# tesseract-robotics/trajopt

Hardware: NVIDIA H100
Metric: converged trajectories/sec (7-DOF x 30 wp, batch 1024) (higher is better)
Workload: dtype f64

## Files before the change

### trajopt_b200/csrc/kernels.h

```cpp
#pragma once
#include "device_types.cuh"

namespace tb200 {
struct EvalExtra;
struct SolveCtl;
using SolveKernelFn = void (*)(DevProblem, EvalExtra, SolveCtl);
using EvalKernelFn = void (*)(DevProblem, EvalExtra, int, const double*);
SolveKernelFn solve_kernel_for(int D, bool pair_rows, bool sing);
EvalKernelFn eval_kernel_for(int D, bool sing);
int eval_debug_prof(unsigned long long* out, int reset);
constexpr int kQpProfSlots = 32;
int qp_debug_prof(unsigned long long* out, int reset);
}
```

### trajopt_b200/csrc/qp_cta_kernel.cuh

```cuda
#pragma once
#include "device_types.cuh"
#include "joint_terms.cuh"

namespace tb200 {

#ifdef TB200_PROFILE
static __device__ unsigned long long g_prof[32];
#define PROF_T0() const long long prof_t0_ = clock64()
#define PROF_ADD(slot) do { if (q.tid == 0) atomicAdd(&g_prof[slot], (unsigned long long)(clock64() - prof_t0_)); } while (0)
#define PROF_COUNT(slot) do { if (q.tid == 0) atomicAdd(&g_prof[slot], 1ull); } while (0)
#define PROF_ADD2(slot, slot2) do { if (q.tid == 0) { const unsigned long long d_ = clock64() - prof_t0_; \
    atomicAdd(&g_prof[slot], d_); atomicAdd(&g_prof[slot2], d_); } } while (0)
#else
#define PROF_T0()
#define PROF_ADD(slot)
#define PROF_COUNT(slot)
#define PROF_ADD2(slot, slot2)
#endif
#if defined(TB200_PROFILE) && defined(TB200_PROFILE_CHECK)
#define PROF_CHK_T0() long long pc_ = clock64()
#define PROF_CHK(slot) do { const long long n_ = clock64(); if (q.tid == 0) atomicAdd(&g_prof[slot], (unsigned long long)(n_ - pc_)); pc_ = n_; } while (0)
#else
#define PROF_CHK_T0()
#define PROF_CHK(slot)
#endif

constexpr int kQpThreads = 256;
constexpr int kQpThreadsC = 256;
constexpr double kOsqpInf = 1e30;
constexpr double kMinScaling = 1e-4, kMaxScaling = 1e4;
constexpr double kVerifyTol = 1e-9;
constexpr int kVerifyRounds = 3;
constexpr double kRhoMin = 1e-6, kRhoMax = 1e6, kRhoTol = 1e-4, kRhoEqOverIneq = 1e3;
enum { QPS_UNSOLVED = 0, QPS_SOLVED = 1, QPS_SOLVED_INACC = 2, QPS_PINF = 3, QPS_PINF_INACC = 4, QPS_DINF = 5,
       QPS_DINF_INACC = 6, QPS_MAXITER = 7, QPS_NONCVX = 8 };

__device__ __forceinline__ double limit_scaling(double v) {
  v = v < kMinScaling ? 1.0 : v;
  return v > kMaxScaling ? kMaxScaling : v;
}
// ... 1441 lines not shown
      }
      v_x = xn;
      v_z = zn;
      v_y += dy;
    }
    __syncthreads();
    PROF_ADD(3);
  }
  if (has_var) {
    q.x[vi] = v_x;
    q.zb[vi] = v_z;
    q.yb[vi] = v_y;
  }
  __syncthreads();
}

template <int NB, int PAIR>
__device__ __noinline__ void admm_block_pinv(const QpCtx& q, const double rho_aux_in, const int n_iter, const int keep_last) {
  constexpr int CNc = PAIR ? ((NB > 3) ? NB : 3) : ((NB / 2 > 3) ? NB / 2 : 3);
  constexpr int kPre = 8;
  constexpr int QN = 3 * NB;
  constexpr int kRowThreads = 64;
  extern __shared__ double sm[];
#ifdef TB200_PROFILE
  const long long prof_entry_ = clock64();
#endif
  const int tid = q.tid, N = q.N, Np = q.Np, nrows = q.nrows, RS = q.RS;
  const double sigma = q.sigma, alpha = q.alpha, oma = 1.0 - q.alpha, rho = q.rho, rho_eq = q.rho_eq, rho_aux = rho_aux_in;
  const double inv_rho_aux = 1.0 / rho_aux, inv_rho = 1.0 / rho, inv_rho_eq = 1.0 / rho_eq;
  double* const v1 = sm + (q.v1 - q.smbase);
  double* const w = sm + (q.w - q.smbase);
  double* const rows = sm + (q.rows - q.smbase);
  const int* const rints = reinterpret_cast<const int*>(sm + (reinterpret_cast<const double*>(q.rints) - q.smbase));
  const int* const colent = reinterpret_cast<const int*>(sm + (reinterpret_cast<const double*>(q.colent) - q.smbase));
  double* const dxs = q.scratch;
  double* const dyb = q.scratch + Np;
  const int M = q.M, PR = q.pl.PR, nS = q.pl.nS, ZS = q.pl.ZS, HO = q.pl.HO, WS = q.pl.WS;
  const double* const fbase = sm + (q.SA - q.smbase);
  const bool upper = tid >= kQpThreads - kRowThreads;
  const bool prow = tid < PR;
  const int pp = prow ? tid / QN : 0, plr = prow ? tid % QN : 0;
  const int pb0 = pp * 4 * NB, pvar = pb0 + plr;
  const int pn = ((M - 4 * pp) < 3 ? (M - 4 * pp) : 3) * NB;
  const int xl_off = (pp > 0) ? (4 * pp - 1) * NB : 0;
  const int xr_off = (4 * pp + 3 < M) ? (4 * pp + 3) * NB : 0;
  const unsigned a_wrow = smem_u32(fbase + q.pl.wo + (prow ? tid : 0) * WS);
  const unsigned a_b = smem_u32(v1 + pb0), a_xl = smem_u32(w + xl_off), a_xr = smem_u32(w + xr_off);
  const bool swork = tid >= PR && tid < PR + 2 * nS;
  const int sw = swork ? tid - PR : 0, srow = sw >> 1, half = sw & 1;
// ... 61 lines not shown
      const double xt = w[vi];
      const double xn = alpha * xt + oma * v_x;
      const double zr = alpha * (v_beta * xt) + oma * v_z;
      double zn = zr + v_y * v_irb;
      zn = fmin(fmax(zn, v_lb), v_ub);
      const double dy = v_rb * (zr - zn);
      if (keep_steps) {
        v_dx = xn - v_x;
        v_dy = dy;
        dxs[vi] = v_dx;
        dyb[vi] = v_dy;
      }
      v_x = xn;
      v_z = zn;
      v_y += dy;
    }
  };

  if (!upper) {
    double pi[QN];
#pragma unroll
    for (int j = 0; j < QN; ++j) pi[j] = prow ? q.pi_g[j * PR + tid] : 0.0;
    bar();
#ifdef TB200_PROFILE
    if (tid == 0) atomicAdd(&g_prof[21], (unsigned long long)(clock64() - prof_entry_));
#endif
    for (int it = 0; it < n_iter; ++it) {
      const bool keep_steps = keep_last && it == n_iter - 1;
      { PROF_T0(); build_rhs(); PROF_ADD(1); }
      {
        PROF_T0();
        PROF_CHK_T0();
        bar();
        PROF_CHK(4);
        double y = 0.0;
        if (prow) {
          double y0 = 0.0, y1 = 0.0;
#pragma unroll
          for (int j = 0; j < QN; j += 2) {
            double2 bb = make_double2(0.0, 0.0);
            if (j < pn) bb = lds_v2_at(a_b + j * 8);
            y0 += pi[j] * bb.x;
            y1 += pi[j + 1] * bb.y;
          }
          y = y0 + y1;
        }
        sep_half();
        PROF_CHK(14);
        bar();
        PROF_CHK(15);
        if (prow) {
          double t0 = 0.0, t1 = 0.0;
#pragma unroll
          for (int t = 0; t < NB; t += 2) {
            const double2 wl = lds_v2_at(a_wrow + t * 8), wr = lds_v2_at(a_wrow + (NB + t) * 8);
            const double2 xl = lds_v2_at(a_xl + t * 8), xr = lds_v2_at(a_xr + t * 8);
            t0 += wl.x * xl.x + wr.x * xr.x;
            t1 += wl.y * xl.y + wr.y * xr.y;
          }
          w[pvar] = y - (t0 + t1);
        }
        bar();
        PROF_CHK(9);
        PROF_ADD(2);
      }
      {
        PROF_T0();
        var_update(keep_steps);
        bar();
        PROF_ADD(3);
      }
    }
  } else {
    for (int r = kQpThreads - 1 - tid; r < nrows; r += kRowThreads)
      admm_row_entry<CNc>(rows + r * RS, rows + r * RS + 2 * CNc, sigma, rho_aux);
    bar();
    for (int it = 0; it < n_iter; ++it) {
      const bool keep_steps = keep_last && it == n_iter - 1;
      build_rhs();
      bar();
      sep_half();
      bar();
      bar();
      for (int r = kQpThreads - 1 - tid; r < nrows; r += kRowThreads)
        admm_row_update<CNc>(rows + r * RS, rows + r * RS + 2 * CNc, rints + r * RI_NINTS, w, sigma, alpha, oma, rho_aux,
                             inv_rho_aux);
      var_update(keep_steps);
      bar();
    }
  }
  if (has_var) {
    q.x[vi] = v_x;
    q.zb[vi] = v_z;
    q.yb[vi] = v_y;
// ... 37 lines not shown
    static_assert(CHK_PA0 == 14 && CHK_DA1 == 18, "vals[] follows ChkQ");
    __syncwarp();
#pragma unroll
    for (int k = 0; k < kChkHash; ++k) {
      double v = vals[k];
      if ((kChkSumMask >> k) & 1u) {
#pragma unroll
        for (int off = 16; off > 0; off >>= 1) v += __shfl_xor_sync(0xffffffffu, v, off);
      } else {
        v = warp_max_norm(v);
      }
      vals[k] = v;
    }
    for (int off = 16; off > 0; off >>= 1) h += __shfl_xor_sync(0xffffffffu, h, off);
    if ((tid & 31) == 0) {
      double* const chk = sm + (q.tmp - q.smbase);
      const int wid = tid >> 5;
#pragma unroll
      for (int k = 0; k < kChkHash; ++k) chk[k * 8 + wid] = vals[k];
      reinterpret_cast<unsigned long long*>(chk + kChkHash * 8)[wid] = h;
    }
    __syncthreads();
  }
}

enum SoaF { S_U0 = 0, S_U1, S_B0, S_B1, S_LO, S_UP, S_QA0, S_QA1, S_WRR, S_IWRR, S_G0, S_G1, S_IDEN, S_UPA0, S_UPA1,
            S_Z, S_Y, S_XA0, S_XA1, S_ZA0, S_ZA1, S_YA0, S_YA1, S_RA0, S_RA1, S_AS };
__host__ __device__ inline size_t qp_soa_doubles(int max_rows, int CN) {
  const size_t rsd = (static_cast<size_t>(max_rows) + 31) & ~static_cast<size_t>(31);
  return rsd * (S_AS + CN) + (rsd * (3 + CN) + 1) / 2 + static_cast<size_t>(max_rows) * CN + 8;
}
template <int NB, int PAIR>
__device__ __noinline__ void admm_block_soa(const QpCtx& q, const double rho_aux_in, const int n_iter, const int keep_last) {
  constexpr int CNc = PAIR ? ((NB > 3) ? NB : 3) : ((NB / 2 > 3) ? NB / 2 : 3);
  const int N = q.N, Np = q.Np, tid = q.tid, nrows = q.nrows;
  const double sigma = q.sigma, alpha = q.alpha, oma = 1.0 - q.alpha, rho = q.rho, rho_eq = q.rho_eq, rho_aux = rho_aux_in;
  const double inv_rho_aux = 1.0 / rho_aux, inv_rho = 1.0 / rho, inv_rho_eq = 1.0 / rho_eq;
  double* const dxs = q.scratch;
  double* const dyb = q.scratch + Np;
  const int RSd = (nrows + 31) & ~31;
  double* const sd = q.soa;
  int* const si = reinterpret_cast<int*>(sd + static_cast<size_t>(RSd) * (S_AS + CNc));
  double* const ct = sd + static_cast<size_t>(RSd) * (S_AS + CNc) + (static_cast<size_t>(RSd) * (3 + CNc) + 1) / 2 + 1;
  const int nnz = q.colptr[Np];
  PROF_T0();
  for (int i = tid; i < N; i += kQpThreads)
// ... 116 lines not shown
      const double xt = q.w[i];
      const double xn = alpha * xt + oma * q.x[i];
      const double zr = alpha * (beta * xt) + oma * q.zb[i];
      double zn = zr + q.yb[i] * irb;
      zn = fmin(fmax(zn, lb), ub);
      const double dy = rb * (zr - zn);
      if (keep_steps) {
        dxs[i] = xn - q.x[i];
        dyb[i] = dy;
      }
      q.x[i] = xn;
      q.zb[i] = zn;
      q.yb[i] += dy;
    }
    __syncthreads();
    PROF_SOA(3);
  }
}

__device__ inline void qp_scale(QpCtx& q, const QpSettings& st, int n_aux_total) {
  double *qs = q.qs, *lbs = q.lbs, *ubs = q.ubs;
  const int N = q.N, tid = q.tid, HB = 2 * q.D, W = HB + 1;
  double* Eb = q.zb;
  q.c = 1.0;
  for (int i = tid; i < q.Np; i += kQpThreads) {
    q.Dz[i] = 1.0;
    Eb[i] = 1.0;
  }
  for (int r = tid; r < q.nrows; r += kQpThreads) {
    double* F = q.F(r);
    F[R_E] = F[R_DA0] = F[R_DA1] = F[R_EA0] = F[R_EA1] = 1.0;
  }
  __syncthreads();
  for (int pass = 0; pass < st.scaling; ++pass) {
    for (int r = tid; r < q.nrows; r += kQpThreads) {
      double* R = q.R(r);
      double* F = q.F(r);
      const int* I = q.I(r);
      const int base = I[RI_BASE], cnt = I[RI_CNT], stride = I[RI_STRIDE], aux = I[RI_AUX];
      const double E = F[R_E];
      double rn = 0.0;
      for (int k = 0; k < cnt; ++k) rn = fmax(rn, fabs(E * R[k] * q.Dz[base + k * stride]));
      double dt0 = 1.0, dt1 = 1.0, et0 = 1.0, et1 = 1.0;
      if (aux >= 1) {
        const double ua = fabs(E * F[R_DA0]), ba = fabs(F[R_EA0] * F[R_DA0]);
        rn = fmax(rn, ua);
        dt0 = 1.0 / sqrt(limit_scaling(fmax(ua, ba)));
        et0 = 1.0 / sqrt(limit_scaling(ba));
      }
      if (aux == 2) {
        const double ua = fabs(E * F[R_DA1]), ba = fabs(F[R_EA1] * F[R_DA1]);
        rn = fmax(rn, ua);
        dt1 = 1.0 / sqrt(limit_scaling(fmax(ua, ba)));
        et1 = 1.0 / sqrt(limit_scaling(ba));
      }
      F[R_RA0] = 1.0 / sqrt(limit_scaling(rn));
      F[R_RA1] = E;
      F[R_DA0] *= dt0;
      F[R_DA1] *= dt1;
      F[R_EA0] *= et0;
      F[R_EA1] *= et1;
    }
    __syncthreads();
    for (int i = tid; i < N; i += kQpThreads) {
      double m = 0.0;
      for (int t = 0; t < q.n_band; ++t) {
        const int k = q.band_offs[t];
        if (k <= i) m = fmax(m, fabs(q.c * q.Dz[i] * q.Pband[i * W + k] * q.Dz[i - k]));
        if (k >= 1 && i + k < N) m = fmax(m, fabs(q.c * q.Dz[i] * q.Pband[(i + k) * W + k] * q.Dz[i + k]));
      }
      const double bn = fabs(Eb[i] * q.Dz[i]);
      m = fmax(m, bn);
      for (int e = q.colptr[i]; e < q.colptr[i + 1]; ++e) {
        const int ent = q.colent[e], r = ent >> 5, k = ent & 31;
        const double* R = q.R(r);
        m = fmax(m, fabs(R[2 * q.CN + R_RA1] * R[k] * q.Dz[i]));
      }
      q.v1[i] = 1.0 / sqrt(limit_scaling(m));
      Eb[i] *= 1.0 / sqrt(limit_scaling(bn));
    }
    __syncthreads();
    for (int i = tid; i < N; i += kQpThreads) q.Dz[i] *= q.v1[i];
    for (int r = tid; r < q.nrows; r += kQpThreads) {
      double* F = q.F(r);
      F[R_E] = F[R_RA1] * F[R_RA0];
    }
    __syncthreads();
    double csum = 0.0, qn = 0.0;
    for (int i = tid; i < N; i += kQpThreads) {
      double m = 0.0;
      for (int t = 0; t < q.n_band; ++t) {
        const int k = q.band_offs[t];
        if (k <= i) m = fmax(m, fabs(q.c * q.Dz[i] * q.Pband[i * W + k] * q.Dz[i - k]));
        if (k >= 1 && i + k < N) m = fmax(m, fabs(q.c * q.Dz[i] * q.Pband[(i + k) * W + k] * q.Dz[i + k]));
      }
      csum += m;
      qn = fmax(qn, fabs(q.c * q.Dz[i] * qs[i]));
    }
    for (int r = tid; r < q.nrows; r += kQpThreads) {
      const double* F = q.F(r);
      const int aux = q.I(r)[RI_AUX];
      if (aux >= 1) qn = fmax(qn, fabs(q.c * F[R_DA0] * F[R_W]));
      if (aux == 2) qn = fmax(qn, fabs(q.c * F[R_DA1] * F[R_W]));
    }
    double red2[2] = {csum, qn};
    block_reduce<2, 0x1u>(q, red2);
    const double mean = limit_scaling(red2[0] / static_cast<double>(N + n_aux_total));
    q.c *= 1.0 / fmax(mean, limit_scaling(red2[1]));
  }
  q.cinv = 1.0 / q.c;
  for (int i = tid; i < q.Np; i += kQpThreads) {
    if (i < N) {
      qs[i] = q.c * q.Dz[i] * qs[i];
      lbs[i] *= Eb[i];
      ubs[i] *= Eb[i];
      q.beta[i] = Eb[i] * q.Dz[i];
    } else {
      qs[i] = 0.0; lbs[i] = -1.0; ubs[i] = 1.0; q.beta[i] = 1.0; q.Dz[i] = 1.0;
    }
  }
  for (int r = tid; r < q.nrows; r += kQpThreads) {
    double* R = q.R(r);
    double* F = q.F(r);
    const int* I = q.I(r);
    const int aux = I[RI_AUX];
    const double E = F[R_E];
    for (int k = 0; k < q.CN; ++k) R[q.CN + k] = E * R[k] * q.Dz[row_var(I, k)];
    F[R_U0] = F[R_U1] = F[R_B0] = F[R_B1] = F[R_QA0] = F[R_QA1] = 0.0;
    F[R_UP] = -F[R_C] * E;
    if (aux == AUX_HINGE) {
      F[R_U0] = -E * F[R_DA0];
// ... 121 lines not shown
    if (has_var) {
      const double xn = v_x + w[vi];
      v_y += v_w * (v_beta * xn - v_bnd);
      v_x = xn;
      xs[vi] = xn;
    }
    __syncthreads();
  }
  return PolishRes{0.0, 0.0, 0.0};
}

template <int NB, int PAIR, bool REGOK>
__device__ inline QpOut qp_solve_block(QpCtx& q, const QpSettings& st, bool warm, double warm_rho,
                                       const double* ws_x, const double* ws_yb, const bool fast_passes) {
  constexpr int CNc = PAIR ? ((NB > 3) ? NB : 3) : ((NB / 2 > 3) ? NB / 2 : 3);
  const int N = q.N, tid = q.tid;
  QpOut out{QPS_UNSOLVED, 0, 0, st.rho, 0, 0, 0, 0, 0, -1, 0, 0};
  double rho;
  double eps_scale;
  int iter, round;
  q.sigma = st.sigma;
  q.alpha = st.alpha;
  {
    rho = warm ? warm_rho : st.rho;
    rho = fmin(fmax(rho, kRhoMin), kRhoMax);
    eps_scale = 1.0;
    iter = 0;
    round = 0;
    q.rho = rho;
    q.rho_eq = kRhoEqOverIneq * rho;
    if (warm) {
      for (int i = tid; i < q.Np; i += kQpThreads) {
        if (i < N) {
          q.x[i] = ws_x[i] / q.Dz[i];
          q.yb[i] = ws_yb[i] * q.Dz[i] / q.beta[i] * q.c;
          q.zb[i] = q.beta[i] * q.x[i];
        } else {
          q.x[i] = q.yb[i] = q.zb[i] = 0.0;
        }
      }
      __syncthreads();
      for (int r = tid; r < q.nrows; r += kQpThreads) {
        double* R = q.R(r);
        double* F = q.F(r);
        const int naux = q.I(r)[RI_AUX];
        F[R_XA0] = (naux >= 1) ? F[R_XA0] / F[R_DA0] : 0.0;
        F[R_XA1] = (naux == 2) ? F[R_XA1] / F[R_DA1] : 0.0;
        F[R_Y] = F[R_Y] / F[R_E] * q.c;
        F[R_YA0] = (naux >= 1) ? F[R_YA0] / F[R_EA0] * q.c : 0.0;
        F[R_YA1] = (naux == 2) ? F[R_YA1] / F[R_EA1] * q.c : 0.0;
        F[R_Z] = row_dot<CNc>(q, R, q.I(r), q.x) + F[R_U0] * F[R_XA0] + F[R_U1] * F[R_XA1];
        F[R_ZA0] = F[R_B0] * F[R_XA0];
        F[R_ZA1] = F[R_B1] * F[R_XA1];
      }
    } else {
      for (int i = tid; i < q.Np; i += kQpThreads) q.x[i] = q.zb[i] = q.yb[i] = 0.0;
      for (int r = tid; r < q.nrows; r += kQpThreads) {
        double* F = q.F(r);
        F[R_XA0] = F[R_XA1] = F[R_Z] = F[R_Y] = F[R_ZA0] = F[R_ZA1] = F[R_YA0] = F[R_YA1] = 0.0;
      }
    }
    __syncthreads();
  }
  SysW sysw{false, st.sigma, rho};
  bool factor_ok = true;

  const QpPlan plan = qp_plan(REGOK, q.pinv, q.rows_smem, q.M, NB, fast_passes);
  const bool use_reg = plan.use_reg;
  const bool use_pinv = plan.use_pinv;
  using BlockFn = void (*)(const QpCtx&, double, int, int);
  const bool fuse = plan.fuse;
  const bool fast_polish = plan.fast_polish;
  bool fused_chk = false;
  auto run_block = [&](int n, bool keep_last) {
    fused_chk = fuse && keep_last;
    if constexpr (REGOK) {
      if (use_pinv || use_reg) {
        BlockFn volatile fn = use_pinv ? &admm_block_pinv<NB, PAIR>
                                       : (q.rows_smem ? &admm_block_fast<NB, PAIR> : &admm_block_soa<NB, PAIR>);
        fn(q, sysw.rho_aux, n, keep_last ? (fuse ? 2 : 1) : 0);
        return;
      }
    }
    BlockFn volatile fn = q.rows_smem ? &admm_block<NB, PAIR> : &admm_block_soa<NB, PAIR>;
    fn(q, sysw.rho_aux, n, keep_last ? 1 : 0);
  };
  using FactorFn = bool (*)(const QpCtx&, const SysW&);
  auto factorize = [&](const SysW& wts) -> bool {
    fused_chk = false;
    FactorFn f = &assemble_factor<NB, false, false>;
    if constexpr (NB <= 16) {
      if (fast_passes && __isShared(q.SA)) f = &assemble_factor<NB, false, true>;
    }
    if constexpr (REGOK) {
      if (use_pinv && !wts.polish) f = &assemble_factor<NB, true, false>;
    }
    FactorFn volatile fn = f;
    return fn(q, wts);
  };
  auto stash_z = [&](const bool restore) {
    extern __shared__ double sm[];
    double2* zs = reinterpret_cast<double2*>(sm + (q.SA - q.smbase) + q.pl.zo);
    double2* zg = reinterpret_cast<double2*>(q.z_stash);
// ... 229 lines not shown
            if (factored && verified) {
              early_verified = true;
              out.pol_factor_ok = 1;
              out.pol_pri = p_pri;
              out.pol_dua = p_dua;
              status = QPS_SOLVED;
              stop = true;
            } else {
              PROF_T0();
              failed_guess = pending_guess;
              have_failed_guess = true;
              restore_fn(false);
              if (use_pinv) {
                stash_z(true);
              } else if (!factorize(sysw)) {
                status = QPS_NONCVX;
                stop = true;
              }
              PROF_ADD(19);
            }
          }
        }
        if (!stop && rho_iter) {
          if (!can_check) residuals(true);
          const double pn = s_pri / (fmax(s_z, s_ax) + 1e-10);
          const double dn = s_dua / (fmax(s_q, fmax(s_aty, s_px)) + 1e-10);
          double rho_new = rho * sqrt(pn / (dn + 1e-10));
          rho_new = fmin(fmax(rho_new, kRhoMin), kRhoMax);
          if (rho_new > rho * st.adaptive_rho_tolerance || rho_new < rho / st.adaptive_rho_tolerance) {
            rho = rho_new;
            q.rho = rho;
            q.rho_eq = kRhoEqOverIneq * rho;
            sysw.rho_aux = rho;
            out.rho_updates++;
            PROF_T0();
            if (!factorize(sysw)) {
              status = QPS_NONCVX;
              stop = true;
            }
            PROF_ADD(20);
          }
        }
      }
    }
  };

  const double wp = 1.0 / st.delta;
  const SysW pw{true, st.delta, 0.0};
  auto polish_refine = [&](bool& verified, double& p_pri, double& p_dua) {
    PROF_T0();
    if constexpr (REGOK) {
// ... 172 lines not shown
      if (factored && verified) {
        out.polish = 1;
        done = true;
      } else if (round >= kVerifyRounds || iter >= st.max_iter) {
        const bool ok = factored && ((p_pri < pri_res && p_dua < dua_res) || (p_pri < pri_res && dua_res < 1e-10) ||
                                     (p_dua < dua_res && pri_res < 1e-10)) && isfinite(p_pri) && isfinite(p_dua);
        out.polish = ok ? 2 : -1;
        done = true;
      } else {
        ++round;
        eps_scale *= 0.1;
        PROF_T0();
        restore_admm_state(false);
        if (use_pinv) {
          stash_z(true);
        } else if (!factorize(sysw)) {
          status = QPS_NONCVX;
          done = true;
        }
        PROF_ADD(19);
      }
    }
  }
  out.iters = iter;
  out.status = status;
  out.rho = rho;
  out.c = q.c;
  if (out.polish != 0) {
    if (out.polish > 0) {
      for (int r = tid; r < q.nrows; r += kQpThreads) {
        double* F = q.F(r);
        for (int k = 0; k < 2; ++k) F[R_XA0 + k] = F[R_PX0 + k];
      }
    }
    restore_admm_state(out.polish > 0);
  }
  return out;
}

static __device__ __noinline__ int qp_singularity_row(const DevProblem& p, const QpCtx& q, const DevObj& o, const int oi,
                                                      const bool is_cnt, const double w_aux, const double* cart_err,
                                                      const double* cart_jac, const int nr, const int n_aux, int* sh_i) {
  const int D = q.D;
  if (q.tid == 0) {
    double* R = q.R(nr);
    int* I = q.rints + static_cast<size_t>(nr) * RI_NINTS;
    const double* J = cart_jac + static_cast<size_t>(o.src_off) * p.cart_stride;
    const double thr = 1e-7 * fabs(o.coeff);
    double dot = 0.0;
    int nz = 0;
    for (int j = 0; j < q.CN; ++j) {
      const double Jj = (j < D) ? J[j] : 0.0;
      dot += Jj * q.x[o.first * D + min(j, D - 1)];
      const double a = (fabs(Jj) > thr) ? Jj : 0.0;
      R[j] = a;
      nz += (a != 0.0);
    }
    R[2 * q.CN + R_C] = cart_err[o.src_off] - dot;
    R[2 * q.CN + R_W] = w_aux;
    I[RI_BASE] = o.first * D; I[RI_CNT] = D; I[RI_STRIDE] = 1; I[RI_AUX] = is_cnt ? AUX_HINGE : AUX_ABS;
    I[RI_OBJ] = oi; I[RI_PAD] = n_aux;
    sh_i[0] = nz;
  }
  __syncthreads();
  const int nz = sh_i[0];
  __syncthreads();
  return nz + (is_cnt ? 1 : 2);
}

template <int DD, int PAIR, int SING = 0>
__device__ __noinline__ void qp_step(const DevProblem& p, const int b, const double* x_override ,
                                        const double* trust_override, int* admm_iters_out, int* polish_out) {
  constexpr int NB = 2 * DD;
  constexpr bool FG = DD > 8;
  extern __shared__ double sm[];
  const int tid = threadIdx.x;
  if (!x_override && (p.status[b] != 5 || p.qp_done[b] != 0)) return;
  const int N = p.N, T = p.T, D = p.D;
  QpCtx q;
  q.N = N; q.T = T; q.D = D; q.tid = tid;
  q.nb = NB;
  q.M = qp_block_count(N, NB);
  q.Np = q.M * NB;
  q.CN = (p.row_stride - R_NF) / 3;
  q.RS = p.row_stride;
  const QpSmem S = qp_smem_layout(N, NB, q.RS, q.CN, p.max_rows, FG);
  if (FG || !S.factor_smem) {
    double* fg = p.factor_g + static_cast<size_t>(blockIdx.x) * qp_cta_global_doubles(N, NB);
    const int fb = qp_even(q.M * NB * NB);
    q.SA = fg; q.SLM = fg + fb; q.SU = fg + 2 * fb;
  } else {
    q.SA = sm + S.SA; q.SLM = sm + S.SLM; q.SU = sm + S.SU;
  }
  q.beta = sm + S.beta;
  q.x = sm + S.x; q.zb = sm + S.zb; q.yb = sm + S.yb; q.v1 = sm + S.v1; q.w = sm + S.w;
  q.qs = sm + S.qs; q.lbs = sm + S.lbs; q.ubs = sm + S.ubs; q.tmp = sm + S.tmp; q.red = sm + S.red;
  q.flag = sm + S.red - 8;
  q.colptr = reinterpret_cast<int*>(sm + S.colptr);
  double* const rows_g = p.rows + static_cast<size_t>(b) * p.max_rows * p.row_stride;
  int* const rints_g = p.row_ints + static_cast<size_t>(b) * p.max_rows * RI_NINTS;
// ... 9 lines not shown
  int* mylist = p.lists + static_cast<size_t>(b) * p.list_stride;
  int* colptr = mylist;
  int* colent = mylist + q.Np + 1;
  int* obj_start = colent + static_cast<size_t>(p.max_rows) * q.CN;
  q.colent = colent;
  q.band_offs = p.band_offs;
  q.n_band = p.n_band;
  if (S.pband_smem) {
    q.Pband = sm + S.Pb;
    for (int t = tid; t < N * (NB + 1); t += kQpThreads) sm[S.Pb + t] = p.Pband[t];
  } else {
    q.Pband = p.Pband;
  }
  double* gvec = p.scratch + static_cast<size_t>(b) * 5 * q.Np;
  q.scratch = gvec;
  q.Dz = sm + S.Dz;
  q.v2 = sm + S.v2;
  double *qs = q.qs, *lbs = q.lbs, *ubs = q.ubs;
  int* meta = p.ws_meta + static_cast<size_t>(b) * 8;
  const int n_obj = p.n_costs + p.n_cnts;
  int nr = 0, n_aux = 0, nnzA = 0;
  bool warm = false;
  int* sh_i = reinterpret_cast<int*>(q.flag + 2);

  {
    const double* xc = (x_override ? x_override : p.x) + static_cast<size_t>(b) * N;
    const double trust = trust_override ? trust_override[b] : p.trust[b];
    const double* mu = p.merit_coeffs + static_cast<size_t>(b) * p.n_cnts;
    const int buf = x_override ? 0 : p.cur_buf[b];
    const size_t slot = static_cast<size_t>(buf) * p.B + b;
    const double* cart_err = p.cart_err + slot * p.n_cart_rows;
    const double* cart_jac = p.cart_jac + slot * static_cast<size_t>(p.n_cart_rows) * p.cart_stride;
    const double* coll_rows = p.coll_rows + slot * static_cast<size_t>(p.n_coll_cand) * p.coll_stride;
    const unsigned long long* coll_mask = p.coll_mask + slot * static_cast<size_t>(p.n_coll_objs) * p.coll_words;

    for (int i = tid; i < N; i += kQpThreads) {
      const double lb = p.lower[i % D], ub = p.upper[i % D];
      const double xi = fmin(fmax(xc[i], lb), ub);
      lbs[i] = fmax(fmax(xi - trust, lb), -kOsqpInf);
      ubs[i] = fmin(fmin(xi + trust, ub), kOsqpInf);
      qs[i] = p.qlin[i];
      q.x[i] = xc[i];
    }
    __syncthreads();

    for (int f = tid; f < p.n_fixed; f += kQpThreads) {
      const int var = p.fixed_vars[f];
      double* R = q.R(f);
      int* I = q.rints + static_cast<size_t>(f) * RI_NINTS;
      for (int k = 0; k < q.CN; ++k) R[k] = (k == 0) ? 1.0 : 0.0;
      R[2 * q.CN + R_C] = -p.init_traj[static_cast<size_t>(b) * N + var];
      R[2 * q.CN + R_W] = 0.0;
      I[RI_BASE] = var; I[RI_CNT] = 1; I[RI_STRIDE] = D; I[RI_AUX] = AUX_NONE; I[RI_OBJ] = -1; I[RI_PAD] = 0;
    }
    nr += p.n_fixed;
    nnzA += p.n_fixed;
    int coll_obj_counter = 0;
    for (int oi = 0; oi < n_obj; ++oi) {
      const bool is_cnt = oi >= p.n_costs;
      const DevObj o = is_cnt ? p.cnt_objs[oi - p.n_costs] : p.cost_objs[oi];
      if (tid == 0) obj_start[oi] = nr;
      const double w_aux = is_cnt ? mu[oi - p.n_costs] : 1.0;
      if (o.kind == OBJ_JOINT_EQ_COST) continue;
      if (o.kind == OBJ_JOINT_EQ_CNT || o.kind == OBJ_JOINT_INEQ_CNT || o.kind == OBJ_JOINT_INEQ_COST) {
        const DevJointTerm& jt = p.joint_terms[o.term];
        const int per = (o.kind == OBJ_JOINT_EQ_CNT) ? 1 : 2;
        const int total = o.n_steps * D * per;
        const double wst[3][3] = {{1, 0, 0}, {-1, 1, 0}, {1, -2, 1}};
        for (int k = tid; k < total; k += kQpThreads) {
          const int t = o.first + k / (D * per), d = (k / per) % D, side = k % per;
          double* R = q.R(nr + k);
          int* I = q.rints + static_cast<size_t>(nr + k) * RI_NINTS;
          const double cd = jt.coeffs[d];
          double sgn = cd, cst;
          if (per == 1) cst = -jt.targets[d] * cd;
          else if (side == 0) cst = (-jt.targets[d] - jt.upper[d]) * cd;
          else { sgn = -cd; cst = (jt.lower[d] + jt.targets[d]) * cd; }
          for (int i = 0; i < q.CN; ++i) R[i] = (i <= o.order) ? wst[o.order][i] * sgn : 0.0;
          R[2 * q.CN + R_C] = cst;
          R[2 * q.CN + R_W] = w_aux;
          I[RI_BASE] = t * D + d; I[RI_CNT] = o.order + 1; I[RI_STRIDE] = D;
          I[RI_AUX] = (per == 1) ? AUX_ABS : AUX_HINGE; I[RI_OBJ] = oi;
          I[RI_PAD] = n_aux + k * ((per == 1) ? 2 : 1);
        }
        nr += total;
        n_aux += total * ((per == 1) ? 2 : 1);
        nnzA += total * (o.order + 1 + ((per == 1) ? 2 : 1));
      } else if (o.kind == OBJ_CART_POSE) {
        const DevCartTerm& ct = p.cart_terms[o.term];
        if (tid == 0) sh_i[0] = 0;
        __syncthreads();
        int nz = 0;
        for (int k = tid; k < o.n_rows; k += kQpThreads) {
          double* R = q.R(nr + k);
          int* I = q.rints + static_cast<size_t>(nr + k) * RI_NINTS;
          const double* J = cart_jac + static_cast<size_t>(o.src_off + k) * p.cart_stride;
          const double thr = 1e-7 * fabs(ct.coeff[k]);
          double dot = 0.0;
          for (int j = 0; j < q.CN; ++j) {
            const double Jj = (j < D) ? J[j] : 0.0;
            dot += Jj * q.x[o.first * D + min(j, D - 1)];
            const double a = (fabs(Jj) > thr) ? Jj : 0.0;
            R[j] = a;
            nz += (a != 0.0);
          }
          R[2 * q.CN + R_C] = cart_err[o.src_off + k] - dot;
          R[2 * q.CN + R_W] = w_aux;
          I[RI_BASE] = o.first * D; I[RI_CNT] = D; I[RI_STRIDE] = 1; I[RI_AUX] = AUX_ABS; I[RI_OBJ] = oi;
          I[RI_PAD] = n_aux + 2 * k;
        }
        if (nz) atomicAdd(&sh_i[0], nz);
        __syncthreads();
        nz = sh_i[0];
        __syncthreads();
        nr += o.n_rows;
        n_aux += 2 * o.n_rows;
        nnzA += nz + 2 * o.n_rows;
      } else if (o.kind == OBJ_CART_VEL) {
        if (tid == 0) sh_i[0] = 0;
        __syncthreads();
        int nz = 0;
        const int per = is_cnt ? 1 : 2;
        for (int k = tid; k < 6; k += kQpThreads) {
          double* R = q.R(nr + k);
          int* I = q.rints + static_cast<size_t>(nr + k) * RI_NINTS;
          const double* J = cart_jac + static_cast<size_t>(o.src_off + k) * p.cart_stride;
          double dot = 0.0;
          for (int j = 0; j < q.CN; ++j) {
            const double Jj = (j < 2 * D) ? J[j] : 0.0;
            dot += Jj * q.x[o.first * D + min(j, 2 * D - 1)];
            const double a = (fabs(Jj) > 1e-7) ? Jj : 0.0;
            R[j] = a;
            nz += (a != 0.0);
          }
          R[2 * q.CN + R_C] = cart_err[o.src_off + k] - dot;
          R[2 * q.CN + R_W] = w_aux;
          I[RI_BASE] = o.first * D; I[RI_CNT] = 2 * D; I[RI_STRIDE] = 1; I[RI_AUX] = is_cnt ? AUX_HINGE : AUX_ABS;
          I[RI_OBJ] = oi; I[RI_PAD] = n_aux + per * k;
        }
        if (nz) atomicAdd(&sh_i[0], nz);
        __syncthreads();
        nz = sh_i[0];
        __syncthreads();
        nr += 6;
        n_aux += per * 6;
        nnzA += nz + per * 6;
      } else if (SING != 0 && o.kind == OBJ_SINGULARITY) {
        nnzA += qp_singularity_row(p, q, o, oi, is_cnt, w_aux, cart_err, cart_jac, nr, n_aux, sh_i);
        nr += 1;
        n_aux += is_cnt ? 1 : 2;
      } else if (o.kind == OBJ_COLL || o.kind == OBJ_COLL_CAST) {
        const unsigned long long* mw = coll_mask + static_cast<size_t>(coll_obj_counter) * p.coll_words;
        ++coll_obj_counter;
        if (tid == 0) { sh_i[0] = 0; sh_i[1] = 0; }
        __syncthreads();
        int nz = 0;
        for (int c = tid; c < o.n_rows; c += kQpThreads) {
          const bool act = (mw[c / 64] >> (c % 64)) & 1ull;
          if (act) {
            int before = 0;
            for (int wdx = 0; wdx < c / 64; ++wdx) before += __popcll(mw[wdx]);
            before += __popcll(mw[c / 64] & ((1ull << (c % 64)) - 1ull));
            const int pos = nr + before;
            double* R = q.R(pos);
            int* I = q.rints + static_cast<size_t>(pos) * RI_NINTS;
            const double* cr = coll_rows + static_cast<size_t>(o.src_off + c) * p.coll_stride;
            const int W = (o.kind == OBJ_COLL_CAST) ? 2 * D : D;
            const double thr = (o.kind == OBJ_COLL_CAST) ? 1e-7 : -1.0;
            const double scale = is_cnt ? cr[W + 2] : 1.0;
            double dot = 0.0;
            for (int j = 0; j < q.CN; ++j) {
              const double g = (j < W) ? cr[j] : 0.0;
              dot += g * q.x[o.first * D + min(j, W - 1)];
              const double a = (fabs(g) > thr) ? -g * scale : 0.0;
              R[j] = (j < W) ? a : 0.0;
              nz += (j < W && a != 0.0);
            }
            R[2 * q.CN + R_C] = (cr[W + 1] - cr[W] + dot) * scale;
            R[2 * q.CN + R_W] = is_cnt ? w_aux : cr[W + 2];
            I[RI_BASE] = o.first * D; I[RI_CNT] = W; I[RI_STRIDE] = 1; I[RI_AUX] = AUX_HINGE; I[RI_OBJ] = oi;
            I[RI_PAD] = n_aux + before;
          }
        }
        if (nz) atomicAdd(&sh_i[0], nz);
        __syncthreads();
        nz = sh_i[0];
        int count = 0;
        for (int wdx = 0; wdx < p.coll_words; ++wdx) count += __popcll(mw[wdx]);
        __syncthreads();
        nr += count;
        n_aux += count;
        nnzA += nz + count;
      }
    }
    if (tid == 0) obj_start[n_obj] = nr;
    nnzA += N + n_aux;
    __syncthreads();

    for (int i = tid; i <= q.Np; i += kQpThreads) colptr[i] = 0;
    __syncthreads();
    for (int r = tid; r < nr; r += kQpThreads) {
      const int* I = q.I(r);
      for (int k = 0; k < I[RI_CNT]; ++k) atomicAdd(&colptr[I[RI_BASE] + k * I[RI_STRIDE] + 1], 1);
    }
    __syncthreads();
    if (tid == 0)
      for (int i = 0; i < q.Np; ++i) colptr[i + 1] += colptr[i];
    __syncthreads();
    for (int i = tid; i < N; i += kQpThreads) {
      if (colptr[i + 1] == colptr[i]) continue;
      int pos = colptr[i];
      for (int r = 0; r < nr && pos < colptr[i + 1]; ++r) {
        const int* I = q.I(r);
        const int base = I[RI_BASE], stride = I[RI_STRIDE], cnt = I[RI_CNT];
        const int off = i - base;
        if (off >= 0 && off % stride == 0 && off / stride < cnt) colent[pos++] = (r << 5) | (off / stride);
      }
    }
    __syncthreads();
    q.nrows = nr;
  }
  for (int i = tid; i <= q.Np; i += kQpThreads) q.colptr[i] = colptr[i];
  __syncthreads();
  const bool rows_in_smem = nr <= S.row_cap;
  double* const rows_s = sm + S.rows;
  if (rows_in_smem) {
    int* rints_s = reinterpret_cast<int*>(sm + S.rints);
    int* colent_s = reinterpret_cast<int*>(sm + S.colent);
    for (int t = tid; t < nr * q.RS; t += kQpThreads) rows_s[t] = rows_g[t];
    for (int t = tid; t < nr * RI_NINTS; t += kQpThreads) rints_s[t] = rints_g[t];
    for (int t = tid; t < q.colptr[q.Np]; t += kQpThreads) colent_s[t] = colent[t];
    q.rows = rows_s;
    q.rows_smem = 1;
    q.rints = rints_s;
    q.colent = colent_s;
  }
  __syncthreads();

  warm = !x_override && p.qp.warm_starting && meta[3] == 1 && meta[0] == n_aux && meta[1] == nr && meta[2] == nnzA;
  { PROF_T0(); qp_scale(q, p.qp, n_aux); PROF_ADD(7); }
  __syncthreads();

  PROF_T0();
  QpOut res = qp_solve_block<NB, PAIR, (DD <= 7)>(q, p.qp, warm, p.ws_rho[b], p.ws_x + static_cast<size_t>(b) * N,
                                                  p.ws_yb + static_cast<size_t>(b) * N, p.qp_fast_passes != 0);
  __syncthreads();
  PROF_ADD(8);
#ifdef TB200_PROFILE
  if (tid == 0) atomicAdd(&g_prof[9], 1ull);
#endif

  double* nx = p.new_x + static_cast<size_t>(b) * N;
  for (int i = tid; i < N; i += kQpThreads) {
    const double xu = q.Dz[i] * q.x[i];
    nx[i] = xu;
    q.v1[i] = xu;
    p.ws_x[static_cast<size_t>(b) * N + i] = xu;
    p.ws_yb[static_cast<size_t>(b) * N + i] = q.cinv * (q.beta[i] / q.Dz[i]) * q.yb[i];
  }
  __syncthreads();
  for (int r = tid; r < nr; r += kQpThreads) {
    double* R = q.R(r);
    double* F = q.F(r);
    const int* I = q.I(r);
    const int aux = I[RI_AUX];
    F[R_Y] = q.cinv * F[R_E] * F[R_Y];
    for (int k = 0; k < 2; ++k) {
      F[R_XA0 + k] = (k < aux) ? F[R_DA0 + k] * F[R_XA0 + k] : 0.0;
      F[R_YA0 + k] = (k < aux) ? q.cinv * F[R_EA0 + k] * F[R_YA0 + k] : 0.0;
    }
    double val = F[R_C];
    for (int i = 0; i < I[RI_CNT]; ++i) val += R[i] * q.v1[I[RI_BASE] + i * I[RI_STRIDE]];
    F[R_MV] = (aux == AUX_ABS || aux == AUX_NONE) ? fabs(val) : fmax(val, 0.0);
  }
  __syncthreads();
  for (int oi = tid; oi < n_obj; oi += kQpThreads) {
    const bool is_cnt = oi >= p.n_costs;
    double s = 0.0;
    if (!is_cnt && p.cost_objs[oi].kind == OBJ_JOINT_EQ_COST) s = joint_obj_value(p, p.cost_objs[oi], q.v1);
    for (int r = obj_start[oi]; r < obj_start[oi + 1]; ++r) {
      const double* F = q.F(r);
      if (is_cnt) s += F[R_MV];
      else s += F[R_W] * (F[R_XA0] + F[R_XA1]);
// ... 11 lines not shown
    p.qp_status[b] = cvx;
    meta[0] = n_aux; meta[1] = nr; meta[2] = nnzA; meta[3] = (cvx == 0) ? 1 : 0; meta[4] = 0;
    p.ws_rho[b] = res.rho;
    if (!x_override) {
      p.n_admm_iters[b] += res.iters;
      p.qp_done[b] = 1;
    }
    if (admm_iters_out) admm_iters_out[b] = res.iters;
    if (polish_out) polish_out[b] = res.polish;
    if (p.qp_paths) {
      const QpPlan pl = qp_plan(DD <= 7, q.pinv, q.rows_smem, q.M, NB, p.qp_fast_passes != 0);
      int bits = qp_plan_block(pl, q.rows_smem) | (pl.fuse ? QPP_FUSED_CHECK : 0);
      if (res.pol_factor_ok == 1) bits |= pl.fast_polish ? QPP_POLISH_FAST : QPP_POLISH_GENERIC;
      if (FG || !S.factor_smem) bits |= QPP_FACTOR_GLOBAL;
      if (!S.pband_smem) bits |= QPP_BAND_GLOBAL;
      if (!rows_in_smem) bits |= QPP_ROWS_GLOBAL;
      atomicOr(&p.qp_paths[b], bits);
    }
    double* g = p.dbg + static_cast<size_t>(b) * 16;
    g[0] = res.status; g[1] = res.iters; g[2] = res.polish; g[3] = res.rho; g[4] = res.pri_res; g[5] = res.dua_res;
    g[6] = res.pol_pri; g[7] = res.pol_dua; g[8] = res.c; g[9] = res.pol_factor_ok; g[10] = res.rho_updates;
    g[11] = nr; g[12] = n_aux; g[13] = nnzA; g[14] = warm ? 1 : 0; g[15] = res.rounds;
  }
}

}
```

Baseline: 1466.

## Parallelize QP setup: warp-batched collision rows, scan colptr, atomic colent fill, fused scaling

Under the fast-setup flag, consecutive collision objectives are handled together: a warp ballot finds the run, active-row counts are prefix-summed with shuffles, and each warp fills one objective's rows. The serial colptr prefix sum becomes a warp scan. The O(N*nrows) column-entry search is replaced by an atomic scatter followed by a per-column insertion sort. qp_scale drops barriers by double-buffering Dz and merging the cost-norm pass into the update pass, and the column norm now reads R_E instead of R_RA1, which may change scaling values. Profiling slots are also added.

```diff
diff --git a/trajopt_b200/csrc/kernels.h b/trajopt_b200/csrc/kernels.h
--- a/trajopt_b200/csrc/kernels.h
+++ b/trajopt_b200/csrc/kernels.h
@@ -9,6 +9,6 @@
 SolveKernelFn solve_kernel_for(int D, bool pair_rows, bool sing);
 EvalKernelFn eval_kernel_for(int D, bool sing);
 int eval_debug_prof(unsigned long long* out, int reset);
-constexpr int kQpProfSlots = 32;
+constexpr int kQpProfSlots = 64;
 int qp_debug_prof(unsigned long long* out, int reset);
 }
diff --git a/trajopt_b200/csrc/qp_cta_kernel.cuh b/trajopt_b200/csrc/qp_cta_kernel.cuh
--- a/trajopt_b200/csrc/qp_cta_kernel.cuh
+++ b/trajopt_b200/csrc/qp_cta_kernel.cuh
@@ -5,8 +5,10 @@
 namespace tb200 {
 
 #ifdef TB200_PROFILE
-static __device__ unsigned long long g_prof[32];
+static __device__ unsigned long long g_prof[64];
 #define PROF_T0() const long long prof_t0_ = clock64()
+#define PROF_LAP_T0() long long lap_ = clock64()
+#define PROF_LAP(slot) do { const long long n_ = clock64(); if (threadIdx.x == 0) atomicAdd(&g_prof[slot], (unsigned long long)(n_ - lap_)); lap_ = n_; } while (0)
 #define PROF_ADD(slot) do { if (q.tid == 0) atomicAdd(&g_prof[slot], (unsigned long long)(clock64() - prof_t0_)); } while (0)
 #define PROF_COUNT(slot) do { if (q.tid == 0) atomicAdd(&g_prof[slot], 1ull); } while (0)
 #define PROF_ADD2(slot, slot2) do { if (q.tid == 0) { const unsigned long long d_ = clock64() - prof_t0_; \
@@ -16,6 +18,8 @@
 #define PROF_ADD(slot)
 #define PROF_COUNT(slot)
 #define PROF_ADD2(slot, slot2)
+#define PROF_LAP_T0()
+#define PROF_LAP(slot)
 #endif
 #if defined(TB200_PROFILE) && defined(TB200_PROFILE_CHECK)
 #define PROF_CHK_T0() long long pc_ = clock64()
@@ -1503,9 +1507,7 @@
   constexpr int QN = 3 * NB;
   constexpr int kRowThreads = 64;
   extern __shared__ double sm[];
-#ifdef TB200_PROFILE
-  const long long prof_entry_ = clock64();
-#endif
+  PROF_LAP_T0();
   const int tid = q.tid, N = q.N, Np = q.Np, nrows = q.nrows, RS = q.RS;
   const double sigma = q.sigma, alpha = q.alpha, oma = 1.0 - q.alpha, rho = q.rho, rho_eq = q.rho_eq, rho_aux = rho_aux_in;
   const double inv_rho_aux = 1.0 / rho_aux, inv_rho = 1.0 / rho, inv_rho_eq = 1.0 / rho_eq;
@@ -1613,14 +1615,12 @@
 #pragma unroll
     for (int j = 0; j < QN; ++j) pi[j] = prow ? q.pi_g[j * PR + tid] : 0.0;
     bar();
-#ifdef TB200_PROFILE
-    if (tid == 0) atomicAdd(&g_prof[21], (unsigned long long)(clock64() - prof_entry_));
-#endif
+    PROF_LAP(21);
     for (int it = 0; it < n_iter; ++it) {
       const bool keep_steps = keep_last && it == n_iter - 1;
-      { PROF_T0(); build_rhs(); PROF_ADD(1); }
+      build_rhs();
+      PROF_LAP(1);
       {
-        PROF_T0();
         PROF_CHK_T0();
         bar();
         PROF_CHK(4);
@@ -1653,14 +1653,11 @@
         }
         bar();
         PROF_CHK(9);
-        PROF_ADD(2);
-      }
-      {
-        PROF_T0();
-        var_update(keep_steps);
-        bar();
-        PROF_ADD(3);
-      }
+        PROF_LAP(2);
+      }
+      var_update(keep_steps);
+      bar();
+      PROF_LAP(3);
     }
   } else {
     for (int r = kQpThreads - 1 - tid; r < nrows; r += kRowThreads)
@@ -1744,6 +1741,7 @@
     }
     __syncthreads();
   }
+  PROF_LAP(41);
 }
 
 enum SoaF { S_U0 = 0, S_U1, S_B0, S_B1, S_LO, S_UP, S_QA0, S_QA1, S_WRR, S_IWRR, S_G0, S_G1, S_IDEN, S_UPA0, S_UPA1,
@@ -1906,9 +1904,10 @@
   double *qs = q.qs, *lbs = q.lbs, *ubs = q.ubs;
   const int N = q.N, tid = q.tid, HB = 2 * q.D, W = HB + 1;
   double* Eb = q.zb;
+  SmVec Dz = q.Dz, Dzn = q.v2;
   q.c = 1.0;
   for (int i = tid; i < q.Np; i += kQpThreads) {
-    q.Dz[i] = 1.0;
+    Dz[i] = 1.0;
     Eb[i] = 1.0;
   }
   for (int r = tid; r < q.nrows; r += kQpThreads) {
@@ -1924,7 +1923,7 @@
       const int base = I[RI_BASE], cnt = I[RI_CNT], stride = I[RI_STRIDE], aux = I[RI_AUX];
       const double E = F[R_E];
       double rn = 0.0;
-      for (int k = 0; k < cnt; ++k) rn = fmax(rn, fabs(E * R[k] * q.Dz[base + k * stride]));
+      for (int k = 0; k < cnt; ++k) rn = fmax(rn, fabs(E * R[k] * Dz[base + k * stride]));
       double dt0 = 1.0, dt1 = 1.0, et0 = 1.0, et1 = 1.0;
       if (aux >= 1) {
         const double ua = fabs(E * F[R_DA0]), ba = fabs(F[R_EA0] * F[R_DA0]);
@@ -1945,44 +1944,40 @@
       F[R_EA0] *= et0;
       F[R_EA1] *= et1;
     }
-    __syncthreads();
     for (int i = tid; i < N; i += kQpThreads) {
       double m = 0.0;
       for (int t = 0; t < q.n_band; ++t) {
         const int k = q.band_offs[t];
-        if (k <= i) m = fmax(m, fabs(q.c * q.Dz[i] * q.Pband[i * W + k] * q.Dz[i - k]));
-        if (k >= 1 && i + k < N) m = fmax(m, fabs(q.c * q.Dz[i] * q.Pband[(i + k) * W + k] * q.Dz[i + k]));
-      }
-      const double bn = fabs(Eb[i] * q.Dz[i]);
+        if (k <= i) m = fmax(m, fabs(q.c * Dz[i] * q.Pband[i * W + k] * Dz[i - k]));
+        if (k >= 1 && i + k < N) m = fmax(m, fabs(q.c * Dz[i] * q.Pband[(i + k) * W + k] * Dz[i + k]));
+      }
+      const double bn = fabs(Eb[i] * Dz[i]);
       m = fmax(m, bn);
       for (int e = q.colptr[i]; e < q.colptr[i + 1]; ++e) {
         const int ent = q.colent[e], r = ent >> 5, k = ent & 31;
         const double* R = q.R(r);
-        m = fmax(m, fabs(R[2 * q.CN + R_RA1] * R[k] * q.Dz[i]));
+        m = fmax(m, fabs(R[2 * q.CN + R_E] * R[k] * Dz[i]));
       }
       q.v1[i] = 1.0 / sqrt(limit_scaling(m));
       Eb[i] *= 1.0 / sqrt(limit_scaling(bn));
     }
     __syncthreads();
-    for (int i = tid; i < N; i += kQpThreads) q.Dz[i] *= q.v1[i];
+    double csum = 0.0, qn = 0.0;
+    for (int i = tid; i < N; i += kQpThreads) {
+      const double di = Dz[i] * q.v1[i];
+      Dzn[i] = di;
+      double m = 0.0;
+      for (int t = 0; t < q.n_band; ++t) {
+        const int k = q.band_offs[t];
+        if (k <= i) m = fmax(m, fabs(q.c * di * q.Pband[i * W + k] * (Dz[i - k] * q.v1[i - k])));
+        if (k >= 1 && i + k < N) m = fmax(m, fabs(q.c * di * q.Pband[(i + k) * W + k] * (Dz[i + k] * q.v1[i + k])));
+      }
+      csum += m;
+      qn = fmax(qn, fabs(q.c * di * qs[i]));
+    }
     for (int r = tid; r < q.nrows; r += kQpThreads) {
       double* F = q.F(r);
       F[R_E] = F[R_RA1] * F[R_RA0];
-    }
-    __syncthreads();
-    double csum = 0.0, qn = 0.0;
-    for (int i = tid; i < N; i += kQpThreads) {
-      double m = 0.0;
-      for (int t = 0; t < q.n_band; ++t) {
-        const int k = q.band_offs[t];
-        if (k <= i) m = fmax(m, fabs(q.c * q.Dz[i] * q.Pband[i * W + k] * q.Dz[i - k]));
-        if (k >= 1 && i + k < N) m = fmax(m, fabs(q.c * q.Dz[i] * q.Pband[(i + k) * W + k] * q.Dz[i + k]));
-      }
-      csum += m;
-      qn = fmax(qn, fabs(q.c * q.Dz[i] * qs[i]));
-    }
-    for (int r = tid; r < q.nrows; r += kQpThreads) {
-      const double* F = q.F(r);
       const int aux = q.I(r)[RI_AUX];
       if (aux >= 1) qn = fmax(qn, fabs(q.c * F[R_DA0] * F[R_W]));
       if (aux == 2) qn = fmax(qn, fabs(q.c * F[R_DA1] * F[R_W]));
@@ -1991,6 +1986,13 @@
     block_reduce<2, 0x1u>(q, red2);
     const double mean = limit_scaling(red2[0] / static_cast<double>(N + n_aux_total));
     q.c *= 1.0 / fmax(mean, limit_scaling(red2[1]));
+    const SmVec t = Dz;
+    Dz = Dzn;
+    Dzn = t;
+  }
+  if (Dz.off != q.Dz.off) {
+    for (int i = tid; i < N; i += kQpThreads) q.Dz[i] = Dz[i];
+    __syncthreads();
   }
   q.cinv = 1.0 / q.c;
   for (int i = tid; i < q.Np; i += kQpThreads) {
@@ -2158,6 +2160,7 @@
   q.sigma = st.sigma;
   q.alpha = st.alpha;
   {
+    PROF_T0();
     rho = warm ? warm_rho : st.rho;
     rho = fmin(fmax(rho, kRhoMin), kRhoMax);
     eps_scale = 1.0;
@@ -2197,6 +2200,7 @@
       }
     }
     __syncthreads();
+    PROF_ADD(39);
   }
   SysW sysw{false, st.sigma, rho};
   bool factor_ok = true;
@@ -2214,7 +2218,9 @@
       if (use_pinv || use_reg) {
         BlockFn volatile fn = use_pinv ? &admm_block_pinv<NB, PAIR>
                                        : (q.rows_smem ? &admm_block_fast<NB, PAIR> : &admm_block_soa<NB, PAIR>);
+        PROF_T0();
         fn(q, sysw.rho_aux, n, keep_last ? (fuse ? 2 : 1) : 0);
+        PROF_ADD(46);
         return;
       }
     }
@@ -2490,11 +2496,13 @@
           }
         }
         if (!stop && rho_iter) {
+          PROF_T0();
           if (!can_check) residuals(true);
           const double pn = s_pri / (fmax(s_z, s_ax) + 1e-10);
           const double dn = s_dua / (fmax(s_q, fmax(s_aty, s_px)) + 1e-10);
           double rho_new = rho * sqrt(pn / (dn + 1e-10));
           rho_new = fmin(fmax(rho_new, kRhoMin), kRhoMax);
+          PROF_ADD(40);
           if (rho_new > rho * st.adaptive_rho_tolerance || rho_new < rho / st.adaptive_rho_tolerance) {
             rho = rho_new;
             q.rho = rho;
@@ -2713,6 +2721,7 @@
       }
     }
   }
+  PROF_T0();
   out.iters = iter;
   out.status = status;
   out.rho = rho;
@@ -2726,6 +2735,7 @@
     }
     restore_admm_state(out.polish > 0);
   }
+  PROF_ADD(42);
   return out;
 }
 
@@ -2767,6 +2777,10 @@
   extern __shared__ double sm[];
   const int tid = threadIdx.x;
   if (!x_override && (p.status[b] != 5 || p.qp_done[b] != 0)) return;
+#ifdef TB200_PROFILE
+  const long long prof_step_ = clock64();
+#endif
+  PROF_LAP_T0();
   const int N = p.N, T = p.T, D = p.D;
   QpCtx q;
   q.N = N; q.T = T; q.D = D; q.tid = tid;
@@ -2822,6 +2836,8 @@
   int nr = 0, n_aux = 0, nnzA = 0;
   bool warm = false;
   int* sh_i = reinterpret_cast<int*>(q.flag + 2);
+  const bool fast_setup = p.qp_fast_passes != 0;
+  int nz_coll = 0;
 
   {
     const double* xc = (x_override ? x_override : p.x) + static_cast<size_t>(b) * N;
@@ -2842,7 +2858,9 @@
       qs[i] = p.qlin[i];
       q.x[i] = xc[i];
     }
+    if (tid == 0) sh_i[3] = 0;
     __syncthreads();
+    PROF_LAP(32);
 
     for (int f = tid; f < p.n_fixed; f += kQpThreads) {
       const int var = p.fixed_vars[f];
@@ -2886,6 +2904,7 @@
         nr += total;
         n_aux += total * ((per == 1) ? 2 : 1);
         nnzA += total * (o.order + 1 + ((per == 1) ? 2 : 1));
+        PROF_LAP(33);
       } else if (o.kind == OBJ_CART_POSE) {
         const DevCartTerm& ct = p.cart_terms[o.term];
         if (tid == 0) sh_i[0] = 0;
@@ -2916,6 +2935,7 @@
         nr += o.n_rows;
         n_aux += 2 * o.n_rows;
         nnzA += nz + 2 * o.n_rows;
+        PROF_LAP(34);
       } else if (o.kind == OBJ_CART_VEL) {
         if (tid == 0) sh_i[0] = 0;
         __syncthreads();
@@ -2945,43 +2965,89 @@
         nr += 6;
         n_aux += per * 6;
         nnzA += nz + per * 6;
+        PROF_LAP(34);
       } else if (SING != 0 && o.kind == OBJ_SINGULARITY) {
         nnzA += qp_singularity_row(p, q, o, oi, is_cnt, w_aux, cart_err, cart_jac, nr, n_aux, sh_i);
         nr += 1;
         n_aux += is_cnt ? 1 : 2;
+        PROF_LAP(34);
       } else if (o.kind == OBJ_COLL || o.kind == OBJ_COLL_CAST) {
+        auto coll_row = [&](const DevObj& oc, const int oci, const bool cnt_c, const double w_c,
+                            const unsigned long long* mw, const int c, const int row0, const int aux0) -> int {
+          int before = 0;
+          for (int wdx = 0; wdx < c / 64; ++wdx) before += __popcll(mw[wdx]);
+          before += __popcll(mw[c / 64] & ((1ull << (c % 64)) - 1ull));
+          const int pos = row0 + before;
+          double* R = q.R(pos);
+          int* I = q.rints + static_cast<size_t>(pos) * RI_NINTS;
+          const double* cr = coll_rows + static_cast<size_t>(oc.src_off + c) * p.coll_stride;
+          const int W = (oc.kind == OBJ_COLL_CAST) ? 2 * D : D;
+          const double thr = (oc.kind == OBJ_COLL_CAST) ? 1e-7 : -1.0;
+          const double scale = cnt_c ? cr[W + 2] : 1.0;
+          double dot = 0.0;
+          int nzr = 0;
+          for (int j = 0; j < q.CN; ++j) {
+            const double g = (j < W) ? cr[j] : 0.0;
+            dot += g * q.x[oc.first * D + min(j, W - 1)];
+            const double a = (fabs(g) > thr) ? -g * scale : 0.0;
+            R[j] = (j < W) ? a : 0.0;
+            nzr += (j < W && a != 0.0);
+          }
+          R[2 * q.CN + R_C] = (cr[W + 1] - cr[W] + dot) * scale;
+          R[2 * q.CN + R_W] = cnt_c ? w_c : cr[W + 2];
+          I[RI_BASE] = oc.first * D; I[RI_CNT] = W; I[RI_STRIDE] = 1; I[RI_AUX] = AUX_HINGE; I[RI_OBJ] = oci;
+          I[RI_PAD] = aux0 + before;
+          return nzr;
+        };
+        if (fast_setup) {
+          const int lane = tid & 31, wid = tid >> 5;
+          const int oj = oi + lane;
+          bool coll = false;
+          if (oj < n_obj) {
+            const int kj = (oj >= p.n_costs) ? p.cnt_objs[oj - p.n_costs].kind : p.cost_objs[oj].kind;
+            coll = kj == OBJ_COLL || kj == OBJ_COLL_CAST;
+          }
+          const unsigned stop = __ballot_sync(0xffffffffu, !coll);
+          const int len = stop ? __ffs(stop) - 1 : 32;
+          int cnt = 0;
+          if (lane < len) {
+            const unsigned long long* mw = coll_mask + static_cast<size_t>(coll_obj_counter + lane) * p.coll_words;
+            for (int wdx = 0; wdx < p.coll_words; ++wdx) cnt += __popcll(mw[wdx]);
+          }
+          int incl = cnt;
+#pragma unroll
+          for (int off = 1; off < 32; off <<= 1) {
+            const int v = __shfl_up_sync(0xffffffffu, incl, off);
+            if (lane >= off) incl += v;
+          }
+          const int excl = incl - cnt;
+          const int total = __shfl_sync(0xffffffffu, incl, 31);
+          if (tid < len) obj_start[oi + tid] = nr + excl;
+          for (int j = wid; j < len; j += kQpThreads / 32) {
+            const int ocj = oi + j;
+            const bool cnt_j = ocj >= p.n_costs;
+            const DevObj oc = cnt_j ? p.cnt_objs[ocj - p.n_costs] : p.cost_objs[ocj];
+            const double w_j = cnt_j ? mu[ocj - p.n_costs] : 1.0;
+            const int start = __shfl_sync(0xffffffffu, excl, j);
+            const unsigned long long* mw = coll_mask + static_cast<size_t>(coll_obj_counter + j) * p.coll_words;
+            for (int c = lane; c < oc.n_rows; c += 32)
+              if ((mw[c / 64] >> (c % 64)) & 1ull) nz_coll += coll_row(oc, ocj, cnt_j, w_j, mw, c, nr + start, n_aux + start);
+          }
+          coll_obj_counter += len;
+          oi += len - 1;
+          nr += total;
+          n_aux += total;
+          nnzA += total;
+          PROF_LAP(35);
+          continue;
+        }
         const unsigned long long* mw = coll_mask + static_cast<size_t>(coll_obj_counter) * p.coll_words;
         ++coll_obj_counter;
         if (tid == 0) { sh_i[0] = 0; sh_i[1] = 0; }
         __syncthreads();
         int nz = 0;
-        for (int c = tid; c < o.n_rows; c += kQpThreads) {
-          const bool act = (mw[c / 64] >> (c % 64)) & 1ull;
-          if (act) {
-            int before = 0;
-            for (int wdx = 0; wdx < c / 64; ++wdx) before += __popcll(mw[wdx]);
-            before += __popcll(mw[c / 64] & ((1ull << (c % 64)) - 1ull));
-            const int pos = nr + before;
-            double* R = q.R(pos);
-            int* I = q.rints + static_cast<size_t>(pos) * RI_NINTS;
-            const double* cr = coll_rows + static_cast<size_t>(o.src_off + c) * p.coll_stride;
-            const int W = (o.kind == OBJ_COLL_CAST) ? 2 * D : D;
-            const double thr = (o.kind == OBJ_COLL_CAST) ? 1e-7 : -1.0;
-            const double scale = is_cnt ? cr[W + 2] : 1.0;
-            double dot = 0.0;
-            for (int j = 0; j < q.CN; ++j) {
-              const double g = (j < W) ? cr[j] : 0.0;
-              dot += g * q.x[o.first * D + min(j, W - 1)];
-              const double a = (fabs(g) > thr) ? -g * scale : 0.0;
-              R[j] = (j < W) ? a : 0.0;
-              nz += (j < W && a != 0.0);
-            }
-            R[2 * q.CN + R_C] = (cr[W + 1] - cr[W] + dot) * scale;
-            R[2 * q.CN + R_W] = is_cnt ? w_aux : cr[W + 2];
-            I[RI_BASE] = o.first * D; I[RI_CNT] = W; I[RI_STRIDE] = 1; I[RI_AUX] = AUX_HINGE; I[RI_OBJ] = oi;
-            I[RI_PAD] = n_aux + before;
-          }
-        }
+        for (int c = tid; c < o.n_rows; c += kQpThreads)
+          if ((mw[c / 64] >> (c % 64)) & 1ull) nz += coll_row(o, oi, is_cnt, w_aux, mw, c, nr, n_aux);
         if (nz) atomicAdd(&sh_i[0], nz);
         __syncthreads();
         nz = sh_i[0];
@@ -2991,11 +3057,15 @@
         nr += count;
         n_aux += count;
         nnzA += nz + count;
+        PROF_LAP(35);
       }
     }
     if (tid == 0) obj_start[n_obj] = nr;
     nnzA += N + n_aux;
+    if (nz_coll) atomicAdd(&sh_i[3], nz_coll);
     __syncthreads();
+    nnzA += sh_i[3];
+    PROF_LAP(35);
 
     for (int i = tid; i <= q.Np; i += kQpThreads) colptr[i] = 0;
     __syncthreads();
@@ -3004,20 +3074,60 @@
       for (int k = 0; k < I[RI_CNT]; ++k) atomicAdd(&colptr[I[RI_BASE] + k * I[RI_STRIDE] + 1], 1);
     }
     __syncthreads();
-    if (tid == 0)
+    if (fast_setup) {
+      if (tid < 32) {
+        int carry = 0;
+        for (int i0 = 0; i0 <= q.Np; i0 += 32) {
+          const int i = i0 + tid;
+          int v = (i <= q.Np) ? colptr[i] : 0;
+#pragma unroll
+          for (int off = 1; off < 32; off <<= 1) {
+            const int u = __shfl_up_sync(0xffffffffu, v, off);
+            if (tid >= off) v += u;
+          }
+          v += carry;
+          if (i <= q.Np) colptr[i] = v;
+          carry = __shfl_sync(0xffffffffu, v, 31);
+        }
+      }
+    } else if (tid == 0) {
       for (int i = 0; i < q.Np; ++i) colptr[i + 1] += colptr[i];
+    }
     __syncthreads();
-    for (int i = tid; i < N; i += kQpThreads) {
-      if (colptr[i + 1] == colptr[i]) continue;
-      int pos = colptr[i];
-      for (int r = 0; r < nr && pos < colptr[i + 1]; ++r) {
+    PROF_LAP(36);
+    if (fast_setup) {
+      int* const cur = reinterpret_cast<int*>(q.v2.ptr());
+      for (int i = tid; i < N; i += kQpThreads) cur[i] = colptr[i];
+      __syncthreads();
+      for (int r = tid; r < nr; r += kQpThreads) {
         const int* I = q.I(r);
         const int base = I[RI_BASE], stride = I[RI_STRIDE], cnt = I[RI_CNT];
-        const int off = i - base;
-        if (off >= 0 && off % stride == 0 && off / stride < cnt) colent[pos++] = (r << 5) | (off / stride);
+        for (int k = 0; k < cnt; ++k) colent[atomicAdd(&cur[base + k * stride], 1)] = (r << 5) | k;
+      }
+      __syncthreads();
+      for (int i = tid; i < N; i += kQpThreads) {
+        const int e0 = colptr[i], e1 = colptr[i + 1];
+        for (int e = e0 + 1; e < e1; ++e) {
+          const int v = colent[e];
+          int f = e;
+          for (; f > e0 && colent[f - 1] > v; --f) colent[f] = colent[f - 1];
+          colent[f] = v;
+        }
+      }
+    } else {
+      for (int i = tid; i < N; i += kQpThreads) {
+        if (colptr[i + 1] == colptr[i]) continue;
+        int pos = colptr[i];
+        for (int r = 0; r < nr && pos < colptr[i + 1]; ++r) {
+          const int* I = q.I(r);
+          const int base = I[RI_BASE], stride = I[RI_STRIDE], cnt = I[RI_CNT];
+          const int off = i - base;
+          if (off >= 0 && off % stride == 0 && off / stride < cnt) colent[pos++] = (r << 5) | (off / stride);
+        }
       }
     }
     __syncthreads();
+    PROF_LAP(37);
     q.nrows = nr;
   }
   for (int i = tid; i <= q.Np; i += kQpThreads) q.colptr[i] = colptr[i];
@@ -3038,14 +3148,15 @@
   __syncthreads();
 
   warm = !x_override && p.qp.warm_starting && meta[3] == 1 && meta[0] == n_aux && meta[1] == nr && meta[2] == nnzA;
-  { PROF_T0(); qp_scale(q, p.qp, n_aux); PROF_ADD(7); }
-  __syncthreads();
-
-  PROF_T0();
+  PROF_LAP(38);
+  qp_scale(q, p.qp, n_aux);
+  PROF_LAP(7);
+  __syncthreads();
+
   QpOut res = qp_solve_block<NB, PAIR, (DD <= 7)>(q, p.qp, warm, p.ws_rho[b], p.ws_x + static_cast<size_t>(b) * N,
                                                   p.ws_yb + static_cast<size_t>(b) * N, p.qp_fast_passes != 0);
   __syncthreads();
-  PROF_ADD(8);
+  PROF_LAP(8);
 #ifdef TB200_PROFILE
   if (tid == 0) atomicAdd(&g_prof[9], 1ull);
 #endif
@@ -3059,6 +3170,7 @@
     p.ws_yb[static_cast<size_t>(b) * N + i] = q.cinv * (q.beta[i] / q.Dz[i]) * q.yb[i];
   }
   __syncthreads();
+  PROF_LAP(43);
   for (int r = tid; r < nr; r += kQpThreads) {
     double* R = q.R(r);
     double* F = q.F(r);
@@ -3116,6 +3228,10 @@
     g[6] = res.pol_pri; g[7] = res.pol_dua; g[8] = res.c; g[9] = res.pol_factor_ok; g[10] = res.rho_updates;
     g[11] = nr; g[12] = n_aux; g[13] = nnzA; g[14] = warm ? 1 : 0; g[15] = res.rounds;
   }
-}
-
-}
+  PROF_LAP(44);
+#ifdef TB200_PROFILE
+  if (tid == 0) atomicAdd(&g_prof[45], (unsigned long long)(clock64() - prof_step_));
+#endif
+}
+
+}
```

After: 1485 (median of 6 runs). 1.3% higher.
